# intellerce/controlanimate

Measured on AMD Instinct MI355X. Metric: frames_per_sec, higher is better.
Workload: dtype fp16

## Files before the change

### controlanimate_amd/attention.py

```python
from __future__ import annotations

from typing import Optional

import torch
from torch import nn

from . import kernels as K
from .attention_processor import Attention, AttnProcessor2_0
from .context import ExecCtx, dispatch
from .layers import HipConv1x1, HipGroupNorm, HipLayerNorm, HipLinear, LnFold, WeightArena, _f32, geglu_interleave, ln_fold_enabled


class GEGLU(nn.Module):
    def __init__(self, dim_in: int, dim_out: int):
        super().__init__()
        self.dim_in, self.dim_out = dim_in, dim_out
        self.proj = HipLinear(dim_in, dim_out * 2)
        self.w = self.b = None

    def pack(self, arena: WeightArena, dtype):
        self.w = arena.add((2 * self.dim_out, self.dim_in), dtype, lambda: geglu_interleave(_f32(self.proj.weight)))
        self.b = arena.add((2 * self.dim_out,), torch.float32, lambda: geglu_interleave(_f32(self.proj.bias)))

    def run(self, x: torch.Tensor) -> torch.Tensor:
        return K.gemm(x, self.w.t, bias=self.b.t, geglu=True)


class FeedForward(nn.Module):
    def __init__(self, dim: int, dim_out: Optional[int] = None, mult: int = 4, dropout: float = 0.0,
                 activation_fn: str = "geglu", final_dropout: bool = False):
        super().__init__()
        if activation_fn != "geglu":
            raise NotImplementedError(activation_fn)
        inner = int(dim * mult)
        self.net = nn.ModuleList([GEGLU(dim, inner), nn.Identity(), HipLinear(inner, dim_out or dim)])

    def pack(self, arena, dtype, fold_ln=None):
        self.fold = None
        if fold_ln is not None and ln_fold_enabled():
            self.fold = LnFold(arena, dtype, fold_ln, [self.net[0].proj], geglu=True)
        else:
            self.net[0].pack(arena, dtype)
        self.net[2].pack(arena, dtype)
        self.w2f = None
        out = self.net[2]
        if self.fold is not None and self.fold.w.frag is not None and (out.out_features, out.in_features) == (320, 1280):
            from .layers import frag_order2
            self.w2f = arena.add((320, 1280), dtype, lambda: frag_order2(out.weight.detach().float()))

    def run_with_proj_out(self, x: torch.Tensor, residual: Optional[torch.Tensor], proj_frag, proj_bias, proj_residual) -> Optional[torch.Tensor]:
        fold = getattr(self, "fold", None)
        if fold is None or getattr(self, "w2f", None) is None or proj_frag is None or not dispatch.attn_out_fused:
            return None
        return K.ff_fused(x, fold.w.frag[0].t, fold.b.t, fold.cs.t, self.w2f.t, None if self.net[2].b is None else self.net[2].b.t,
                          fold.eps, residual=residual, w_out_frag=proj_frag.t, bias_out=None if proj_bias is None else proj_bias.t,
                          residual_out=proj_residual)

    def run(self, x: torch.Tensor, residual: Optional[torch.Tensor] = None, sums=None) -> torch.Tensor:
        fold = getattr(self, "fold", None)
        if fold is not None and getattr(self, "w2f", None) is not None and sums is None:
            y = K.ff_fused(x, fold.w.frag[0].t, fold.b.t, fold.cs.t, self.w2f.t, None if self.net[2].b is None else self.net[2].b.t,
                           fold.eps, residual=residual)
            if y is not None:
                return y
        if fold is not None:
            h = K.gemm(x, fold.w.t, bias=fold.b.t, geglu=True, ln=(K.RowStats(x, fold.eps, sums), fold.cs.t))
        else:
            h = self.net[0].run(x)
        return self.net[2].run(h, residual=residual)


class BasicTransformerBlock(nn.Module):
    def __init__(self, query_dim: int, num_attention_heads: int, attention_head_dim: int, dropout=0.0,
                 cross_attention_dim: Optional[int] = None, activation_fn: str = "geglu", attention_bias: bool = False,
                 upcast_attention: bool = False, unet_use_cross_frame_attention=False, unet_use_temporal_attention=False, **_):
        super().__init__()
        if unet_use_cross_frame_attention or unet_use_temporal_attention:
            raise NotImplementedError("both flags are false in configs/inference/inference-v{1,2}.yaml")
        self.processor = AttnProcessor2_0()
        self.attn1 = Attention(query_dim, heads=num_attention_heads, dim_head=attention_head_dim, bias=attention_bias)
        self.norm1 = HipLayerNorm(query_dim)
        self.attn2 = Attention(query_dim, cross_attention_dim=cross_attention_dim, heads=num_attention_heads,
                               dim_head=attention_head_dim, bias=attention_bias) if cross_attention_dim is not None else None
        self.norm2 = HipLayerNorm(query_dim) if cross_attention_dim is not None else None
        self.ff = FeedForward(query_dim, activation_fn=activation_fn)
        self.norm3 = HipLayerNorm(query_dim)

    def get_processor(self, return_deprecated_lora: bool = False):
        return self.processor

    def set_processor(self, processor, _remove_lora: bool = False):
        if isinstance(getattr(self, "processor", None), nn.Module) and not isinstance(processor, nn.Module):
            self._modules.pop("processor", None)
        self.processor = processor

    def pack(self, arena, dtype):
        self.attn1.pack(arena, dtype, fold_ln=self.norm1)
        self.norm1.pack(arena, dtype)
        if self.attn2 is not None:
            self.attn2.pack(arena, dtype, fold_ln=self.norm2)
            self.norm2.pack(arena, dtype)
        self.ff.pack(arena, dtype, fold_ln=self.norm3)
        self.norm3.pack(arena, dtype)

    def forward(self, x: torch.Tensor, ctx: ExecCtx, proj_out=None) -> torch.Tensor:
        return self.forward_rest(self.forward_self(x), ctx, proj_out=proj_out)

    def forward_self(self, x: torch.Tensor) -> torch.Tensor:
        B, N, C = x.shape
        next_folded = (self.attn2.fold if self.attn2 is not None else self.ff.fold) is not None
        if self.attn1.fold is not None:
            x = self.attn1(x, residual=x, ln=(K.RowStats(x.view(B * N, C), self.norm1.eps, K.row_sums_of(x)), self.attn1.fold),
                           row_sums=next_folded)
        else:
            x = self.attn1(self.norm1.run(x.view(B * N, C)).view(B, N, C), residual=x, row_sums=next_folded)
        return x

    def forward_rest(self, x: torch.Tensor, ctx: ExecCtx, proj_out=None) -> torch.Tensor:
        B, N, C = x.shape
        if self.attn2 is not None:
            kw = dict(encoder_hidden_states=ctx.ehs, residual=x, frames_per_kv=ctx.frames_per_kv, kv_mod=ctx.kv_mod, cache=ctx.cache,
                      row_sums=self.ff.fold is not None)
            if self.attn2.fold is not None:
                x = self.attn2(x, ln=(K.RowStats(x.view(B * N, C), self.norm2.eps, K.row_sums_of(x)), self.attn2.fold), **kw)
            else:
                x = self.attn2(self.norm2.run(x.view(B * N, C)).view(B, N, C), **kw)
        x2 = x.view(B * N, C)
        if self.ff.fold is None:
            return self.ff.run(self.norm3.run(x2), residual=x2).view(B, N, C)
        if proj_out is not None and K.row_sums_of(x) is None:
            y = self.ff.run_with_proj_out(x2, x2, *proj_out)
            if y is not None:
                y = y.view(B, N, C)
                y._proj_out_done = True
                return y
        return self.ff.run(x2, residual=x2, sums=K.row_sums_of(x)).view(B, N, C)


class Transformer3DModel(nn.Module):
    def __init__(self, num_attention_heads: int = 16, attention_head_dim: int = 88, in_channels: Optional[int] = None,
                 num_layers: int = 1, norm_num_groups: int = 32, cross_attention_dim: Optional[int] = None,
                 use_linear_projection: bool = False, **kw):
        super().__init__()
        if use_linear_projection:
            raise NotImplementedError("SD1.5 uses 1x1-conv projections")
        inner = num_attention_heads * attention_head_dim
        self.in_channels = in_channels
        self.norm = HipGroupNorm(norm_num_groups, in_channels, eps=1e-6)
        self.proj_in = HipConv1x1(in_channels, inner)
        self.transformer_blocks = nn.ModuleList([
            BasicTransformerBlock(inner, num_attention_heads, attention_head_dim, cross_attention_dim=cross_attention_dim, **kw)
            for _ in range(num_layers)])
        self.proj_out = HipConv1x1(inner, in_channels)

    def pack(self, arena, dtype):
        self.norm.pack(arena, dtype)
        self.proj_in.pack(arena, dtype)
        for b in self.transformer_blocks:
            b.pack(arena, dtype)
        self.proj_out.pack(arena, dtype)
        self.proj_out_frag = None
        po = self.proj_out
        if tuple(po.weight.shape[:2]) == (320, 320) and getattr(self.transformer_blocks[-1].ff, "w2f", None) is not None:
            from .layers import frag_order_wout
            self.proj_out_frag = arena.add((102400,), dtype, lambda: frag_order_wout(_f32(po.weight).reshape(320, 320)))

    def forward(self, x: torch.Tensor, ctx: ExecCtx, shared_half: bool = False) -> torch.Tensor:
        images, h, w, c = x.shape
        rows = images * h * w
        y = self.norm.run(x)
        y0 = self.proj_in.run(y.view(rows, c), row_sums=self.transformer_blocks[0].attn1.fold is not None)
        y = K.carry_row_sums(y0.view(images, h * w, -1), y0)
        nblk = len(self.transformer_blocks)
        pfrag = getattr(self, "proj_out_frag", None)

        def proj(k, x_rows):
            return (pfrag, self.proj_out.b, x_rows) if (k == nblk - 1 and pfrag is not None) else None
        if shared_half:
            y = self.transformer_blocks[0].forward_self(y)
            y, x = K.repeat_batch(y), K.repeat_batch(x)
            images, rows = 2 * images, 2 * rows
            y = self.transformer_blocks[0].forward_rest(y, ctx, proj_out=proj(0, x.view(rows, c)))
        for k in range(1 if shared_half else 0, nblk):
            y = self.transformer_blocks[k](y, ctx, proj_out=proj(k, x.view(rows, c)))
        if getattr(y, "_proj_out_done", False):
            return y.view(images, h, w, c)
        return self.proj_out.run(y.view(rows, -1), residual=x.view(rows, c)).view(images, h, w, c)
```

### controlanimate_amd/context.py

```python
from __future__ import annotations

from dataclasses import dataclass, field
from typing import Optional

import torch


@dataclass
class ExecCtx:
    b: int
    f: int
    dtype: torch.dtype
    temb: torch.Tensor
    emb_groups: int
    ehs: Optional[torch.Tensor] = None
    frames_per_kv: int = 1
    kv_mod: int = 0
    gn_frames_per_stat: int = 1
    cache: dict = field(default_factory=dict)

    @property
    def images(self) -> int:
        return self.b * self.f

    def rows_per_emb_group(self, h: int, w: int) -> int:
        return self.images // self.emb_groups * h * w


class Dispatch:
    gemm_ar = True
    ff_fused = True
    tattn_fused = True
    xattn_fused = True
    attn_out_fused = True
    xattn_ip_fused = True
    conv_winograd = True
    gn_winograd = True
    conv_up2_phase = True
    ln_row_sums = True
    repeat_kernel = True
    ln_fold = True
    cfg_shared = True
    cn_cfg_dedup = True
    pdc_block_fused = True
    dpt_head_fused = False
    pose_conv7_direct = True
    nbae_refine_fused = True
    controlnet_streams = 2


dispatch = Dispatch()
```

### controlanimate_amd/csrc/ca_gemm_plan.h

```cpp
#pragma once
#include "ca_gemm_core.h"

namespace ca_gemm_detail {

inline unsigned desc_bytes(int64_t elems) {
  const int64_t b = elems * 2;
  return (b > 0 && b < (int64_t)0xFFFFFF00ll) ? (unsigned)b : 0u;
}

inline bool dma_shape_ok(const GemmKParams& p) { return (p.c1 + p.c2) % BK == 0 && (p.c2 == 0 || p.c1 % BK == 0); }
inline bool dma_sizes_ok(const GemmKParams& p) { return p.a_bytes != 0 && p.w_bytes != 0 && (p.c2 == 0 || p.a2_bytes != 0); }
inline bool dma_capable(const GemmKParams& p) { return dma_shape_ok(p) && dma_sizes_ok(p); }

inline bool wres_eligible(const GemmKParams& p) {
  static const int wres_env = CA_KNOB("CA_GEMM_WRES", -1);
  const int kc = p.c1 + p.c2;
  return wres_env != 0 && kc == 320 && p.taps == 1 && (p.c2 == 0 || p.c1 % 32 == 0) && p.n % 160 == 0 && p.n / 160 <= 32 && !p.out_f32 &&
         p.splits <= 1 && !p.ln_parts && dma_sizes_ok(p) &&
         (!p.rowbias || p.rows_per_group % 32 == 0) &&
         act_out_fit31(p) &&
         (wres_env == 1 || p.m >= 16384);
}

inline bool ar_eligible(const GemmKParams& p, bool scratch) {
  static const int ar_env = CA_KNOB("CA_GEMM_AR", -1);
  if (ar_env == 0 || !p.wf || !wres_eligible(p)) return false;
  return p.c2 == 0 && p.n % 64 == 0 && p.alpha == 1.f && p.post == 1.f && p.act == CA_ACT_NONE && !p.row_sums && ((uintptr_t)p.wf & 15) == 0 &&
         ((uintptr_t)p.c & 15) == 0 && p.ldc % 8 == 0 && (!p.res || (((uintptr_t)p.res & 15) == 0 && p.ld_res % 8 == 0 && !p.geglu && !p.ln_colsum)) &&
         (!p.rowbias || (p.rows_per_group % 128 == 0 && !p.geglu)) && (!p.ln_inline || scratch) &&
         (ar_env == 1 || p.n >= 960);
}

struct GemmPlan {
  PlanKind kind;
  int bm, bn, nbuf;
  int splits;
  unsigned tiles;
};

inline bool ps_capable(const GemmKParams& p) {
  const int nt = p.taps * p.kc_tiles;
  const bool fits32 = act_out_fit31(p) && p.w_bytes < FIT31;
  const bool aligned = ((uintptr_t)p.c & 15) == 0 && (!p.res || ((uintptr_t)p.res & 15) == 0) && p.ldc % 8 == 0 && (!p.res || p.ld_res % 8 == 0);
  return dma_capable(p) && p.n % 320 == 0 && nt >= 2 && p.splits <= 1 && !p.out_f32 && !p.ln_inline && (p.ln_parts <= 2 || p.ln_parts == 4) && fits32 && aligned &&
         (!p.rowbias || p.rows_per_group % 64 == 0) && !(p.geglu && (p.res || p.row_sums)) && p.post == 1.f && p.act == CA_ACT_NONE;
}

inline bool pq_capable(const GemmKParams& p, int mode) {
  const bool conv_ok = mode != 1 || (p.pad_lo == 1 && p.ups == 0 && p.hin >= 2 && p.win >= 2 && (int64_t)(p.m / (p.hout * p.wout) + 1) * p.hin * p.win < (1 << 23) &&
                                     (p.hout - 1) * p.stride < p.hin && (p.wout - 1) * p.stride < p.win);
  const bool epi1 = p.geglu || p.ln_colsum || p.ln_stats;
  return ps_capable(p) && (!p.row_sums || (mode == 0 && !epi1)) && (mode == 1 || p.c2 == 0) && (!p.rowbias || p.rows_per_group % 128 == 0) && conv_ok &&
         (!epi1 || (mode == 0 && !p.res && !p.rowbias && p.ln_parts == 0 && (!p.ln_colsum || p.ln_stats)));
}

struct SplitKRule { int env, max_blocks; bool f32_out; };
struct SplitK { int ranges; int64_t bytes; };
inline SplitK splitk_decide(const GemmKParams& p, int mode) {
  static const SplitKRule conv{CA_KNOB("CA_SPLITK", -1), 383, true}, dense{CA_KNOB("CA_SPLITK_DENSE", -1), 192, false};
  const SplitKRule& r = mode == 0 ? dense : conv;
  const SplitK none{1, 0};
  if (!dma_capable(p) || p.ln_inline || p.row_sums || p.ln_parts) return none;
  if (r.env == 0 || p.geglu || (p.out_f32 && !r.f32_out) || p.n % 128 != 0) return none;
  const int nt = p.taps * p.kc_tiles;
  const int64_t blocks = (int64_t)ceil_div_i(p.m, 128) * (p.n / 128);
  if (blocks > r.max_blocks || nt < 48) return none;
  int s = r.env > 0 ? r.env : (int)((960 + blocks - 1) / blocks);
  if (s > 8) s = 8;
  while (s > 1 && nt / s < 12) --s;
  return s > 1 ? SplitK{s, (int64_t)s * p.m * p.n * 4} : none;
}
inline void splitk_apply(const SplitK& k, void* workspace, int64_t workspace_bytes, GemmKParams& p) {
  if (k.ranges > 1 && workspace && workspace_bytes >= k.bytes) {
    p.splits = k.ranges;
    p.partial = reinterpret_cast<float*>(workspace);
  }
}

inline GemmPlan plan_gemm(const GemmKParams& p, int mode) {
  const bool dma = dma_capable(p);
  const int nt = p.taps * p.kc_tiles;
  if (dma && p.splits > 1) {
    static const int pp_split_env = CA_KNOB("CA_SPLITK_PP", 1);
    if (pp_split_env && mode == 0 && p.n % 320 == 0) {
      const int tiles320 = ceil_div_i(p.m, 128) * (p.n / 320);
      int s_eff = 256 / tiles320;
      if (s_eff > p.splits) s_eff = p.splits;
      if (s_eff >= 2 && tiles320 * s_eff >= 128 && nt / s_eff >= 12) {
        return GemmPlan{PK_PP2_SPLITK, 128, 320, 0, s_eff, (unsigned)tiles320};
      }
    }
    return GemmPlan{PK_DMA_SPLITK, 128, 128, 1, p.splits, (unsigned)(ceil_div_i(p.m, 128) * (p.n / 128))};
  }
  static const int pp_env = CA_KNOB("CA_GEMM_PP", -1);
  static const int pq_env = CA_KNOB("CA_GEMM_PQ", -1);
  if (pq_env != 0 && pq_capable(p, mode)) {
    const int64_t tiles = (int64_t)ceil_div_i(p.m, 256) * (p.n / 320);
    const bool dflt = mode == 1 ? (tiles >= 256 && (p.n >= 640 || nt >= 64)) : (tiles >= 256 && (tiles % 256 == 0 || tiles >= 1024) && nt >= 8 && !wres_eligible(p));
    const bool epi1 = p.geglu || p.ln_colsum || p.ln_stats;
    const bool dflt2 = dflt && (mode == 1 || p.geglu), dflt3 = dflt && mode == 1, dflt4 = dflt && (mode == 1 || p.geglu || !epi1);
    if ((pq_env < 0 && dflt) || pq_env == 1 || (pq_env == 2 && dflt2) || (pq_env == 3 && dflt3) || (pq_env == 4 && dflt4) || (pq_env == 5 && dflt)) {
      return GemmPlan{PK_PQ, 256, 320, 0, 1, (unsigned)tiles};
    }
  }
  static const int ps_env = CA_KNOB("CA_GEMM_PS", -1);
  if (ps_env != 0 && ps_capable(p)) {
    const int64_t tiles = (int64_t)ceil_div_i(p.m, 128) * (p.n / 320);
    const bool dflt = mode == 0 && !wres_eligible(p) && nt <= 20 && tiles >= 256 && (p.geglu || p.n <= 1280);
    if ((ps_env < 0 && dflt) || ps_env == 1 || (ps_env == 2 && !(mode == 0 && wres_eligible(p)))) {
      return GemmPlan{PK_PS, 128, 320, 0, 1, (unsigned)tiles};
    }
  }
  if (mode == 0 && dma && ar_eligible(p, p.partial != nullptr)) return GemmPlan{PK_AR, 128, 64, 0, 1, 0u};
  if (mode == 0 && dma && wres_eligible(p)) return GemmPlan{PK_WRES, 256, 160, 0, 1, 0u};
  if (dma && pp_env != 0 && nt >= 2 && p.n % 320 == 0 && p.splits <= 1) {
    const int64_t tiles = (int64_t)ceil_div_i(p.m, 128) * (p.n / 320);
    if (p.row_sums || pp_env == 2 || (pp_env < 0 && tiles >= 128 && nt >= 10 && (tiles <= 256 || (tiles <= 512 && mode == 0)))) {
      return GemmPlan{PK_PP2, 128, 320, 0, 1, (unsigned)tiles};
    }
  }
  const bool wide = p.n % 128 == 0 && (int64_t)ceil_div_i(p.m, 128) * ceil_div_i(p.n, 128) >= 512;
  const int64_t blocks = (int64_t)ceil_div_i(p.m, 128) * ceil_div_i(p.n, wide ? 128 : 64);
  const int nbuf = blocks >= 512 ? 1 : 3;
  if (dma && !wide && p.n % 160 == 0 && (int64_t)ceil_div_i(p.m, 128) * (p.n / 160) >= 512) return GemmPlan{PK_DMA, 128, 160, 1, 1, 0u};
  return GemmPlan{dma ? PK_DMA : PK_REG, 128, wide ? 128 : 64, dma ? nbuf : 2, 1, 0u};
}

inline int row_sums_parts_of(GemmKParams p) {
  p.row_sums = nullptr;
  if (p.geglu || p.out_f32) return 0;
  const PlanKind k = plan_gemm(p, 0).kind;
// ... 236 lines not shown
```

### controlanimate_amd/csrc/ca_gemm_pp.hip

```cpp
#include "ca_gemm_core.h"
#include <type_traits>

namespace {
using namespace ca_gemm_detail;
#include "ca_gemm_pp2.h"
#include "ca_gemm_wres.h"
#include "ca_gemm_ps.h"
#include "ca_gemm_pq.h"

int cu_count() {
  static int n = 0;
  if (!n) {
    int dev = 0;
    hipDeviceProp_t prop;
    if (hipGetDevice(&dev) == hipSuccess && hipGetDeviceProperties(&prop, dev) == hipSuccess) n = prop.multiProcessorCount;
    if (n <= 0) n = 256;
  }
  return n;
}

template <class Launch>
int launch_stamped(const GemmKParams& p, hipStream_t st, const char* label, unsigned sep, unsigned eol, Launch launch) {
  static unsigned long long* dbuf = nullptr;
  if (!dbuf && hipMalloc(&dbuf, 4096 * 8) != hipSuccess) return CA_ERR_LAUNCH;
  (void)hipMemsetAsync(dbuf, 0, 4096 * 8, st);
  GemmKParams q = p;
  q.partial = reinterpret_cast<float*>(dbuf);
  launch(q);
  (void)hipStreamSynchronize(st);
  static int printed = 0;
  if (printed++ < 1) {
    static unsigned long long host[4096];
    (void)hipMemcpy(host, dbuf, sizeof(host), hipMemcpyDeviceToHost);
    for (int g = 0; g < 2; ++g) {
      fprintf(stderr, "[%s stamps group %d, %dx%dx%d] tag:delta_cycles ...\n", label, g, p.m, p.n, (p.c1 + p.c2) * p.taps);
      unsigned long long prev = host[g * 2048];
      for (int i = 0; i < 1000 && host[g * 2048 + 2 * i]; ++i) {
        fprintf(stderr, "%llu:%llu ", host[g * 2048 + 2 * i + 1], host[g * 2048 + 2 * i] - prev);
        prev = host[g * 2048 + 2 * i];
        if (host[g * 2048 + 2 * i + 1] == sep) fprintf(stderr, "| ");
        if (host[g * 2048 + 2 * i + 1] == eol) fprintf(stderr, "\n");
      }
      fprintf(stderr, "\n");
    }
  }
  return CA_OK;
}

template <int DT, int MODE>
int launch_pp(const GemmKParams& p, PlanKind kind, unsigned tiles, hipStream_t st) {
  const unsigned c_bytes = (unsigned)c_extent_bytes(p), res_bytes = (unsigned)res_extent_bytes(p);
  const unsigned grid = tiles < (unsigned)cu_count() ? tiles : (unsigned)cu_count();
  switch (kind) {
    case PK_PQ: {
      auto launch = [&](const GemmKParams& q) {
        if (MODE == 0 && (q.geglu || q.ln_colsum || q.ln_stats)) hipLaunchKernelGGL((k_gemm_pq<DT, 0, 1>), dim3(grid), dim3(512), 0, st, q, (int)tiles, c_bytes, 0u);
        else if (MODE == 0 && q.row_sums) hipLaunchKernelGGL((k_gemm_pq<DT, 0, 2>), dim3(grid), dim3(512), 0, st, q, (int)tiles, c_bytes, res_bytes);
        else hipLaunchKernelGGL((k_gemm_pq<DT, MODE>), dim3(grid), dim3(512), 0, st, q, (int)tiles, c_bytes, res_bytes);
      };
#ifdef CA_STAMPS
      if (p.dbg == 9) return launch_stamped(p, st, "pq", 8, 10, launch);
#endif
      launch(p);
      return CA_OK;
    }
    case PK_PS: {
      auto launch = [&](const GemmKParams& q) { hipLaunchKernelGGL((k_gemm_ps<DT, MODE>), dim3(grid), dim3(512), 0, st, q, (int)tiles, c_bytes, res_bytes); };
#ifdef CA_STAMPS
      if (p.dbg == 9) return launch_stamped(p, st, "ps", 8, 10, launch);
#endif
      launch(p);
      return CA_OK;
    }
    case PK_WRES: {
      if (MODE != 0) return CA_ERR_LAUNCH;
      const int panels = p.n / 160;
      const int chunks = (p.m + 255) / 256;
      int per = (cu_count() / 8) / panels;
      if (per * 8 > chunks) per = chunks / 8;
      if (per < 1) per = 1;
      const unsigned rb_bytes = p.rowbias ? (unsigned)(((int64_t)((p.m - 1) / p.rows_per_group) * p.ld_rowbias + p.n) * 4) : 16u;
      hipLaunchKernelGGL((k_gemm_wres<DT>), dim3(8 * per * panels), dim3(512), 0, st, p, panels, 8 * per, chunks, rb_bytes, c_bytes, res_bytes);
      return CA_OK;
    }
    case PK_PP2:
      hipLaunchKernelGGL((k_gemm_pp2<DT, MODE>), dim3(tiles), dim3(512), 0, st, p);
      return CA_OK;
// ... 21 lines not shown
```

### controlanimate_amd/csrc/ca_gemm_pq.h

```cpp

#ifdef CA_PQ_ABLATE
#define CA_PQ_ABL(bit) (((CA_PQ_ABLATE) & (bit)) != 0)
#else
#define CA_PQ_ABL(bit) false
#endif

__device__ __forceinline__ unsigned pq_udiv(unsigned r, unsigned d, unsigned mag) {
  const unsigned q = __umulhi(r, mag);
  return r - q * d >= d ? q + 1 : q;
}

template <int DT, int MODE, int EPI = 0>
__global__ __launch_bounds__(512, 2) void k_gemm_pq(GemmKParams p, int tiles_total, unsigned c_bytes, unsigned res_bytes) {
  constexpr int BM = 256, BN = 320, KT = 64;
  constexpr int TM = 8, TN = 5;
  constexpr int A_ROWS = 256, B0_ROWS = 128, B1_ROWS = 192;
  constexpr int OFF_A = 0, OFF_B0 = A_ROWS * KT, OFF_B1 = (A_ROWS + B0_ROWS) * KT;
  constexpr int BUF = (A_ROWS + B0_ROWS + B1_ROWS) * KT;
  constexpr int PAR_BASE = 2 * BUF * 2;
  constexpr int P_BI = 0, P_RB0 = 1280, P_RB1 = 2560, P_CS = 3840, PSET = EPI == 1 ? 5120 : 4096;
  constexpr int FLAG_BASE = PAR_BASE + 2 * PSET;
  constexpr int SMEM_BYTES = FLAG_BASE + 8 * 2 * 256;
  static_assert(SMEM_BYTES <= 160 * 1024, "LDS");
  __shared__ __attribute__((aligned(16))) unsigned char smem_b[SMEM_BYTES];
// ... 23 lines not shown
  const bool geglu = EPI == 1 && p.geglu != 0;
  const unsigned long long res_addr = (unsigned long long)(p.res ? (const void*)p.res : (const void*)p.c);
  const u32x4 rs_res = {(unsigned)__builtin_amdgcn_readfirstlane((int)(unsigned)res_addr), (unsigned)__builtin_amdgcn_readfirstlane((int)(unsigned)((res_addr >> 32) & 0xffffu)),
                        (unsigned)__builtin_amdgcn_readfirstlane((int)(p.res ? res_bytes : 0u)), 0x00020000u};
  const unsigned rb_groups = p.rowbias ? (unsigned)((p.m + p.rows_per_group - 1) / p.rows_per_group) : 0u;
  const __amdgpu_buffer_rsrc_t rs_rb = __builtin_amdgcn_make_buffer_rsrc((void*)(p.rowbias ? (const void*)p.rowbias : (const void*)p.w), 0,
                                                                         p.rowbias ? (unsigned)(((int64_t)(rb_groups - 1) * p.ld_rowbias + p.n) * 4) : 0u, 0x00020000);
  const __amdgpu_buffer_rsrc_t rs_seq = __builtin_amdgcn_make_buffer_rsrc((void*)ca_seq_table.v, 0, 4096u, 0x00020000);

#ifdef CA_STAMPS
  unsigned long long* const stamps = reinterpret_cast<unsigned long long*>(p.partial);
  int stamp_i = 0;
  auto stamp = [&](int tag) __attribute__((always_inline)) {
    if (p.dbg == 9 && blockIdx.x == 0 && (wid == 0 || wid == 4) && lane == 0 && stamp_i < 1000) {
      stamps[(wid >> 2) * 2048 + 2 * stamp_i] = __builtin_readcyclecounter();
      stamps[(wid >> 2) * 2048 + 2 * stamp_i + 1] = (unsigned long long)tag;
      ++stamp_i;
    }
  };
#else
  auto stamp = [&](int) __attribute__((always_inline)) {};
#endif
  auto swz = [](int row) { return (row >> 1) & 7; };
  const int kc = p.c1 + p.c2;
  const int kct = kc / KT;
  const unsigned wld = (unsigned)(p.taps * kc);
  const int nt = p.taps * kct;
  const int total_kt = my_tiles * nt;

  constexpr unsigned OOB_V = 0x80000000u;
  unsigned b0_v[2] = {0, 0}, b1_v[3] = {0, 0, 0};
  unsigned a_v[4] = {0, 0, 0, 0};
  int d_seq = 0, d_t = 0, d_tap = 0, d_c0 = 0, d_n = 0;
  bool d_live = true;
  unsigned char* const my_flags = smem_b + FLAG_BASE + wid * 2 * 256;

  auto tile_of = [&](int seq, int& tm, int& tn) __attribute__((always_inline)) -> bool {
    const int id = seq * G + bslot;
    if (id >= tiles_total) return false;
    tile_coords((unsigned)id, tiles_m, tiles_n, tm, tn);
    return true;
  };

  auto dma_set_tile = [&](int seq, int m0, int n0) __attribute__((always_inline)) {
    if (CA_PQ_ABL(16)) m0 = 0, n0 = 0;
    int lane_o = lane;
    asm volatile("" : "+v"(lane_o));
    const int r8 = lane_o >> 3, cp = lane_o & 7;
    const int a_chunk0 = cp ^ swz(r8), b1_chunk0 = cp ^ swz(wid * 24 + r8);
#pragma unroll
    for (int i = 0; i < 4; ++i) {
      const int m = m0 + wid * 32 + i * 8 + r8;
      const bool ok = m < p.m;
      if (MODE == 2) {
        const int ph = m0 / (p.up2_tiles * BM);
        const int py = ph >> 1, px = ph & 1;
        const int r = m - ph * (p.up2_tiles * BM);
        const bool okr = r < p.up2_rows;
        const int rr = okr ? r : p.up2_rows - 1;
        const unsigned q = pq_udiv((unsigned)rr, (unsigned)p.win, p.up2_mag_w);
        const int xs = rr - (int)q * p.win;
        const int ys = (int)q - (int)pq_udiv(q, (unsigned)p.hin, p.up2_mag_h) * p.hin;
        const int hi0 = ys + py - 1, wi0 = xs + px - 1;
        const int p0 = rr + (py - 1) * p.win + (px - 1);
        a_v[i] = ((unsigned)p0 & 0xFFFFFFu) | (hi0 >= 0 ? 1u << 24 : 0u) | (hi0 + 1 < p.hin ? 1u << 25 : 0u) | (wi0 >= 0 ? 1u << 26 : 0u) | (wi0 + 1 < p.win ? 1u << 27 : 0u) |
                 (okr ? 1u << 28 : 0u);
      } else if (MODE == 1) {
        const int mm = ok ? m : p.m - 1;
        const int hw = p.hout * p.wout;
        const int img = mm / hw;
        const int rem = mm - img * hw;
        const int ho = rem / p.wout, wo = rem - ho * p.wout;
        const int hi0 = ho * p.stride - p.pad_lo, wi0 = wo * p.stride - p.pad_lo;
        const int p0 = (img * p.hin + hi0) * p.win + wi0;
        a_v[i] = ((unsigned)p0 & 0xFFFFFFu) | (hi0 >= 0 ? 1u << 24 : 0u) | (hi0 + 2 < p.hin ? 1u << 25 : 0u) | (wi0 >= 0 ? 1u << 26 : 0u) | (wi0 + 2 < p.win ? 1u << 27 : 0u) |
                 (ok ? 1u << 28 : 0u);
      } else {
        a_v[i] = ok ? (unsigned)m * (unsigned)p.lda * 2u + (unsigned)((a_chunk0 ^ (4 * (i & 1))) * 16) : OOB_V;
      }
    }
    unsigned wgrp = 0u;
    if (MODE == 0 && EPI == 0 && p.w_group_rows > 0) wgrp = (unsigned)(m0 / p.w_group_rows) * p.w_group_stride;
    if (MODE == 2) wgrp = (unsigned)(m0 / (p.up2_tiles * BM)) * p.w_group_stride;
#pragma unroll
    for (int i = 0; i < 2; ++i) {
      const int r = wid * 16 + i * 8 + r8;
      b0_v[i] = wgrp + (unsigned)(n0 + (r >> 5) * 80 + ca_ps_col((r >> 4) & 1, r & 15, geglu)) * wld * 2u + (unsigned)((a_chunk0 ^ (4 * i)) * 16);
    }
#pragma unroll
    for (int i = 0; i < 3; ++i) {
      const int r1 = wid * 24 + i * 8 + r8;
      b1_v[i] = wgrp + (unsigned)(n0 + (r1 / 48) * 80 + ca_ps_col(2 + (r1 % 48) / 16, r1 & 15, geglu)) * wld * 2u + (unsigned)((b1_chunk0 ^ (4 * (i & 1))) * 16);
    }
    d_tap = 0;
    d_c0 = 0;
    unsigned char* pset = smem_b + PAR_BASE + (seq & 1) * PSET;
    if (EPI == 1 && wid == 4) {
      const __amdgpu_buffer_rsrc_t rs_cs = __builtin_amdgcn_make_buffer_rsrc((void*)(p.ln_colsum ? (const void*)p.ln_colsum : (const void*)p.w), 0, p.ln_colsum ? (unsigned)p.n * 4u : 0u, 0x00020000);
      __builtin_amdgcn_raw_ptr_buffer_load_lds(rs_cs, (__attribute__((address_space(3))) void*)(pset + P_CS), 16, (unsigned)n0 * 4u + lane_o * 16u, 0, 0, 0);
      __builtin_amdgcn_raw_ptr_buffer_load_lds(rs_cs, (__attribute__((address_space(3))) void*)(pset + P_CS + 1024), 4, (unsigned)n0 * 4u + 1024u + lane_o * 4u, 0, 0, 0);
    }
    if (wid >= 1 && wid <= 3) {
      const bool has1 = p.rowbias && m0 / p.rows_per_group + 1 < (int)rb_groups;
      const unsigned base = wid == 1 ? (unsigned)n0 * 4u
                                     : wid == 2 ? (unsigned)n0 * 4u + (unsigned)(p.rowbias ? m0 / p.rows_per_group : 0) * (unsigned)p.ld_rowbias * 4u
                                                : (has1 ? (unsigned)n0 * 4u + (unsigned)(m0 / p.rows_per_group + 1) * (unsigned)p.ld_rowbias * 4u : OOB_V);
      unsigned char* dst = pset + (wid == 1 ? P_BI : wid == 2 ? P_RB0 : P_RB1);
      if (wid == 1) {
        __builtin_amdgcn_raw_ptr_buffer_load_lds(rs_bi, (__attribute__((address_space(3))) void*)dst, 16, base + lane_o * 16u, 0, 0, 0);
        __builtin_amdgcn_raw_ptr_buffer_load_lds(rs_bi, (__attribute__((address_space(3))) void*)(dst + 1024), 4, base + 1024u + lane_o * 4u, 0, 0, 0);
      } else {
        __builtin_amdgcn_raw_ptr_buffer_load_lds(rs_rb, (__attribute__((address_space(3))) void*)dst, 16, base + lane_o * 16u, 0, 0, 0);
        __builtin_amdgcn_raw_ptr_buffer_load_lds(rs_rb, (__attribute__((address_space(3))) void*)(dst + 1024), 4, base + 1024u + lane_o * 4u, 0, 0, 0);
      }
    }
  };

  auto issue_tile = [&]() __attribute__((always_inline)) {
    if (!d_live) return;
    if (CA_PQ_ABL(1) && d_n >= 2) {
      ++d_n;
      ++d_t;
      return;
    }
    const int par = d_n & 1;
    u16* buf = smem + par * BUF;
    const unsigned wk = (unsigned)(d_tap * kc + d_c0) * 2u;
    const bool src2 = d_c0 >= p.c1;
    __builtin_amdgcn_raw_ptr_buffer_load_lds(rs_w, (__attribute__((address_space(3))) void*)(buf + OFF_B0 + (wid * 2 + 0) * 8 * KT), 16, b0_v[0], wk, 0, 0);
    __builtin_amdgcn_raw_ptr_buffer_load_lds(rs_w, (__attribute__((address_space(3))) void*)(buf + OFF_B0 + (wid * 2 + 1) * 8 * KT), 16, b0_v[1], wk, 0, 0);
    if (MODE != 0) {
      int lane_o = lane;
      asm volatile("" : "+v"(lane_o));
      const unsigned cs2 = (unsigned)(src2 ? p.c2 : p.c1) * 2u;
      const int kh = MODE == 2 ? d_tap >> 1 : (d_tap >= 6 ? 2 : (d_tap >= 3 ? 1 : 0)), kw = MODE == 2 ? d_tap & 1 : d_tap - kh * 3;
      const unsigned need = MODE == 2 ? (1u << 28) | (kh == 0 ? 1u << 24 : 1u << 25) | (kw == 0 ? 1u << 26 : 1u << 27)
                                      : (1u << 28) | (kh == 0 ? 1u << 24 : kh == 2 ? 1u << 25 : 0u) | (kw == 0 ? 1u << 26 : kw == 2 ? 1u << 27 : 0u);
      const int delta = kh * p.win + kw;
      const unsigned cadd = (unsigned)(src2 ? d_c0 - p.c1 : d_c0) * 2u + (unsigned)(((lane_o & 7) ^ swz(lane_o >> 3)) * 16);
#pragma unroll
      for (int i = 0; i < 4; ++i) {
        const unsigned av = a_v[i];
        const int pix = (((int)(av << 8)) >> 8) + delta;
        const unsigned off = __umul24((unsigned)pix, cs2) + (cadd ^ ((i & 1) ? 64u : 0u));
        const unsigned voff = (av & need) == need ? off : OOB_V;
        void* d = buf + OFF_A + (wid * 4 + i) * 8 * KT;
        if (src2) __builtin_amdgcn_raw_ptr_buffer_load_lds(rs_a2, (__attribute__((address_space(3))) void*)d, 16, voff, 0, 0, 0);
        else __builtin_amdgcn_raw_ptr_buffer_load_lds(rs_a, (__attribute__((address_space(3))) void*)d, 16, voff, 0, 0, 0);
      }
    } else {
#pragma unroll
      for (int i = 0; i < 4; ++i)
        __builtin_amdgcn_raw_ptr_buffer_load_lds(rs_a, (__attribute__((address_space(3))) void*)(buf + OFF_A + (wid * 4 + i) * 8 * KT), 16, a_v[i], (unsigned)d_c0 * 2u, 0, 0);
    }
#pragma unroll
    for (int i = 0; i < 3; ++i)
      __builtin_amdgcn_raw_ptr_buffer_load_lds(rs_w, (__attribute__((address_space(3))) void*)(buf + OFF_B1 + (wid * 3 + i) * 8 * KT), 16, b1_v[i], wk, 0, 0);
    __builtin_amdgcn_raw_ptr_buffer_load_lds(rs_seq, (__attribute__((address_space(3))) void*)(my_flags + par * 256), 4, 0u, (unsigned)(d_n & 1023) * 4u, 0, 0);
    ++d_n;
    ++d_t;
    if (p.taps == 1) {
      d_c0 += KT;
    } else if (++d_tap == p.taps) {
      d_tap = 0;
      d_c0 += KT;
    }
  };
#define CA_PQ_SET_TILE(SEQ)                                  \
  {                                                          \
    int tm_, tn_;                                            \
    d_live = tile_of((SEQ), tm_, tn_);                       \
    if (d_live) dma_set_tile((SEQ), tm_ * BM, tn_ * BN);     \
  }
  auto advance_and_issue = [&]() __attribute__((always_inline)) {
    if (d_t == nt) {
      d_t = 0;
      ++d_seq;
      CA_PQ_SET_TILE(d_seq)
    }
    issue_tile();
  };
// ... 305 lines not shown
```

### controlanimate_amd/layers.py

```python
from __future__ import annotations

from typing import Callable, List, Optional, Sequence, Tuple

import torch
from torch import nn

from . import kernels as K
from .context import dispatch

ALIGN = 256


class Packed:

    __slots__ = ("shape", "dtype", "fill", "offset", "t", "frag")

    def __init__(self, shape, dtype, fill):
        self.shape = tuple(int(s) for s in shape)
        self.dtype = dtype
        self.fill = fill
        self.offset = -1
        self.t: Optional[torch.Tensor] = None
        self.frag = None

# ... 242 lines not shown
        def w_cat():
            return torch.cat([_f32(m.weight).reshape(m.weight.shape[0], -1) for m in mods], 0)

        def w_fold():
            w = w_cat() * _f32(ln.weight)[None, :]
            return geglu_interleave(w) if geglu else w

        def bias():
            b = w_cat() @ _f32(ln.bias)
            b = b + torch.cat([_f32(m.bias) if getattr(m, "bias", None) is not None else torch.zeros(m.weight.shape[0], device=m.weight.device) for m in mods], 0)
            return geglu_interleave(b) if geglu else b

        self.w = arena.add((n, k), dtype, w_fold)
        self.w_fold = w_fold
        if frag_wanted(n, k):
            self.w.frag = (arena.add((n, k), dtype, lambda: frag_order(w_fold(), geglu)), geglu)
        self.cs = arena.add((n,), torch.float32, lambda: w_fold().to(dtype).float().sum(1))
        self.b = arena.add((n,), torch.float32, bias)
        self.pe = None
        if pe is not None:
            self.pe = arena.add((pe.shape[-2], n), torch.float32, lambda: _f32(pe).reshape(pe.shape[-2], k).to(mods[0].weight.device) @ w_cat().to(dtype).float().t())
        self._rb_cache = {}

    def rowbias(self, b: int, f: int) -> torch.Tensor:
        if f > self.pe.t.shape[0]:
            raise ValueError(f"video_length {f} exceeds temporal_position_encoding_max_len {self.pe.t.shape[0]}")
        key = (b, f, self.pe.t.data_ptr())
        rb = self._rb_cache.get(key)
        if rb is None:
            rb = self._rb_cache[key] = self.pe.t[:f].repeat(b, 1).contiguous()
        return rb


def geglu_interleave(w: torch.Tensor) -> torch.Tensor:
    d = w.shape[0] // 2
    return torch.stack([w[:d], w[d:]], dim=1).reshape(w.shape)
```

### controlanimate_amd/motion_module.py

```python
from __future__ import annotations

import math

import torch
from torch import nn

from . import kernels as K
from .attention import FeedForward
from .attention_processor import Attention
from .context import ExecCtx
from .layers import HipGroupNorm, HipLayerNorm, HipLinear, WeightArena, _f32


def get_motion_module(in_channels, motion_module_type: str, motion_module_kwargs: dict):
    if motion_module_type == "Vanilla":
        return VanillaTemporalModule(in_channels=in_channels, **motion_module_kwargs)
    raise ValueError(motion_module_type)


class PositionalEncoding(nn.Module):
    def __init__(self, d_model, dropout=0.0, max_len=24):
        super().__init__()
        position = torch.arange(max_len).unsqueeze(1)
        div_term = torch.exp(torch.arange(0, d_model, 2) * (-math.log(10000.0) / d_model))
# ... 29 lines not shown
        no_bias = all(getattr(m, "bias", None) is None for m in (self.to_q, self.to_k, self.to_v))
        if self.fold is not None and pe is not None and no_bias and (self.heads, self.inner_dim, self.query_dim) == (8, 320, 320):
            from .layers import _f32, frag_order_tattn
            self.tfrag = arena.add((368640,), dtype, lambda: frag_order_tattn(torch.cat([_f32(m.weight) for m in (self.to_q, self.to_k, self.to_v)], 0)))
            self.tgamma = arena.add((320,), torch.float32, lambda: _f32(fold_ln.weight))
            self.tbias_pe = arena.add((pe.shape[-2], 320), torch.float32,
                                      lambda: _f32(pe).reshape(pe.shape[-2], 320).to(fold_ln.bias.device) + _f32(fold_ln.bias)[None, :])
            self.tln_eps = fold_ln.eps

    def pos_table(self, frames: int):
        if self.pos_encoder is None:
            return None
        if frames > self.pos_encoder.max_len:
            raise ValueError(f"video_length {frames} exceeds temporal_position_encoding_max_len {self.pos_encoder.max_len}")
        return self.pos_encoder.table.t[:frames]


class TemporalTransformerBlock(nn.Module):
    def __init__(self, dim, num_attention_heads, attention_head_dim, attention_block_types=("Temporal_Self", "Temporal_Self"),
                 dropout=0.0, cross_attention_dim=768, activation_fn="geglu", attention_bias=False, upcast_attention=False,
                 cross_frame_attention_mode=None, temporal_position_encoding=False, temporal_position_encoding_max_len=24, **_):
        super().__init__()
        self.attention_blocks = nn.ModuleList([
            VersatileAttention(attention_mode=name.split("_")[0],
                               cross_attention_dim=cross_attention_dim if name.endswith("_Cross") else None,
                               query_dim=dim, heads=num_attention_heads, dim_head=attention_head_dim, bias=attention_bias,
                               temporal_position_encoding=temporal_position_encoding,
                               temporal_position_encoding_max_len=temporal_position_encoding_max_len)
            for name in attention_block_types])
        self.norms = nn.ModuleList([HipLayerNorm(dim) for _ in attention_block_types])
        self.ff = FeedForward(dim, activation_fn=activation_fn)
        self.ff_norm = HipLayerNorm(dim)

    def pack(self, arena, dtype):
        for attn, norm in zip(self.attention_blocks, self.norms):
            attn.pack(arena, dtype, fold_ln=norm)
            norm.pack(arena, dtype)
        self.ff.pack(arena, dtype, fold_ln=self.ff_norm)
        self.ff_norm.pack(arena, dtype)

    def forward(self, x: torch.Tensor, ctx: ExecCtx, tokens: int, proj_out=None) -> torch.Tensor:
        rows, C = x.shape
        nblk = len(self.attention_blocks)
        for i, (attn, norm) in enumerate(zip(self.attention_blocks, self.norms)):
            nxt = (self.attention_blocks[i + 1].fold if i + 1 < nblk else self.ff.fold) is not None
            if attn.fold is not None:
                o = attn(x.view(1, rows, C), residual=x.view(1, rows, C), temporal=(ctx.b, ctx.f, tokens),
                         ln=(K.RowStats(x, norm.eps, K.row_sums_of(x)), attn.fold), row_sums=nxt)
            else:
                n = norm.run(x, pos=attn.pos_table(ctx.f), rows_per_frame=tokens, frames=ctx.f)
                o = attn(n.view(1, rows, C), residual=x.view(1, rows, C), temporal=(ctx.b, ctx.f, tokens), row_sums=nxt)
            x = K.carry_row_sums(o.view(rows, C), o)
        if self.ff.fold is None:
            return self.ff.run(self.ff_norm.run(x), residual=x)
        if proj_out is not None and K.row_sums_of(x) is None:
            y = self.ff.run_with_proj_out(x, x, *proj_out)
            if y is not None:
                y._proj_out_done = True
                return y
        return self.ff.run(x, residual=x, sums=K.row_sums_of(x))


class TemporalTransformer3DModel(nn.Module):
    def __init__(self, in_channels, num_attention_heads, attention_head_dim, num_layers, norm_num_groups=32, **kw):
        super().__init__()
        inner = num_attention_heads * attention_head_dim
        self.norm = HipGroupNorm(norm_num_groups, in_channels, eps=1e-6)
        self.proj_in = HipLinear(in_channels, inner)
        self.transformer_blocks = nn.ModuleList([
            TemporalTransformerBlock(dim=inner, num_attention_heads=num_attention_heads,
                                     attention_head_dim=attention_head_dim, **kw) for _ in range(num_layers)])
        self.proj_out = HipLinear(inner, in_channels)

    def pack(self, arena, dtype):
        self.norm.pack(arena, dtype)
        self.proj_in.pack(arena, dtype)
        for b in self.transformer_blocks:
            b.pack(arena, dtype)
        self.proj_out.pack(arena, dtype)
        self.proj_out_frag = None
        po = self.proj_out
        if tuple(po.weight.shape) == (320, 320) and getattr(self.transformer_blocks[-1].ff, "w2f", None) is not None:
            from .layers import frag_order_wout
            self.proj_out_frag = arena.add((102400,), dtype, lambda: frag_order_wout(_f32(po.weight)))

    def forward(self, x: torch.Tensor, ctx: ExecCtx) -> torch.Tensor:
        images, h, w, c = x.shape
        rows = images * h * w
        y = self.norm.run(x)
        y = self.proj_in.run(y.view(rows, c), row_sums=self.transformer_blocks[0].attention_blocks[0].fold is not None)
        pfrag = getattr(self, "proj_out_frag", None)
        last = len(self.transformer_blocks) - 1
        for k, blk in enumerate(self.transformer_blocks):
            y = blk(y, ctx, h * w, proj_out=(pfrag, self.proj_out.b, x.view(rows, c)) if (k == last and pfrag is not None) else None)
        if getattr(y, "_proj_out_done", False):
            return y.view(images, h, w, c)
        return self.proj_out.run(y, residual=x.view(rows, c)).view(images, h, w, c)


class VanillaTemporalModule(nn.Module):
    def __init__(self, in_channels, num_attention_heads=8, num_transformer_block=2,
                 attention_block_types=("Temporal_Self", "Temporal_Self"), cross_frame_attention_mode=None,
                 temporal_position_encoding=False, temporal_position_encoding_max_len=24, temporal_attention_dim_div=1,
                 zero_initialize=True):
        super().__init__()
        self.temporal_transformer = TemporalTransformer3DModel(
            in_channels=in_channels, num_attention_heads=num_attention_heads,
            attention_head_dim=in_channels // num_attention_heads // temporal_attention_dim_div,
            num_layers=num_transformer_block, attention_block_types=attention_block_types,
            cross_frame_attention_mode=cross_frame_attention_mode, temporal_position_encoding=temporal_position_encoding,
            temporal_position_encoding_max_len=temporal_position_encoding_max_len)
        if zero_initialize:
            nn.init.zeros_(self.temporal_transformer.proj_out.weight)
            nn.init.zeros_(self.temporal_transformer.proj_out.bias)

    def pack(self, arena, dtype):
        self.temporal_transformer.pack(arena, dtype)

    def forward(self, x: torch.Tensor, ctx: ExecCtx) -> torch.Tensor:
        return self.temporal_transformer(x, ctx)
```

Measured before the change: 16.12.

## Fold feed-forward output linear into transformer proj_out as one two-source GEMM

For the last transformer block, whenever the fused 320-channel path does not apply, the FF output projection and the following proj_out linear are merged algebraically into a single GEMM. It uses weights [Wp·W2 | Wp] over the concatenated inputs (GEGLU output, FF residual) and the folded bias Wp·b2+bp. This drops one full GEMM launch and the round trip of its intermediate activation. To support it, the persistent PQ GEMM kernel gains a second-A-source load path for non-epilogue mode 0, with launch guards and a heuristic gate for two-source cases. The catch is a larger K dimension (inner+C instead of inner) for that GEMM, plus fp16 rounding differences from the premultiplied weights.

```diff
diff --git a/controlanimate_amd/attention.py b/controlanimate_amd/attention.py
--- a/controlanimate_amd/attention.py
+++ b/controlanimate_amd/attention.py
@@ -8,7 +8,7 @@
 from . import kernels as K
 from .attention_processor import Attention, AttnProcessor2_0
 from .context import ExecCtx, dispatch
-from .layers import HipConv1x1, HipGroupNorm, HipLayerNorm, HipLinear, LnFold, WeightArena, _f32, geglu_interleave, ln_fold_enabled
+from .layers import FfProjFold, HipConv1x1, HipGroupNorm, HipLayerNorm, HipLinear, LnFold, WeightArena, _f32, geglu_interleave, ln_fold_enabled
 
 
 class GEGLU(nn.Module):
@@ -35,22 +35,31 @@
         inner = int(dim * mult)
         self.net = nn.ModuleList([GEGLU(dim, inner), nn.Identity(), HipLinear(inner, dim_out or dim)])
 
-    def pack(self, arena, dtype, fold_ln=None):
-        self.fold = None
+    def pack(self, arena, dtype, fold_ln=None, proj_out=None):
+        self.fold = self.pfold = None
         if fold_ln is not None and ln_fold_enabled():
             self.fold = LnFold(arena, dtype, fold_ln, [self.net[0].proj], geglu=True)
         else:
             self.net[0].pack(arena, dtype)
+        out = self.net[2]
+        c320 = self.fold is not None and self.fold.w.frag is not None and (out.out_features, out.in_features) == (320, 1280)
+        if proj_out is not None and self.fold is not None and not c320 and dispatch.ff_proj_fold:
+            self.pfold = FfProjFold(arena, dtype, out, proj_out)
+            out.w = out.b = None
+            self.w2f = None
+            return
         self.net[2].pack(arena, dtype)
         self.w2f = None
-        out = self.net[2]
-        if self.fold is not None and self.fold.w.frag is not None and (out.out_features, out.in_features) == (320, 1280):
+        if c320:
             from .layers import frag_order2
             self.w2f = arena.add((320, 1280), dtype, lambda: frag_order2(out.weight.detach().float()))
 
-    def run_with_proj_out(self, x: torch.Tensor, residual: Optional[torch.Tensor], proj_frag, proj_bias, proj_residual) -> Optional[torch.Tensor]:
+    def run_with_proj_out(self, x: torch.Tensor, residual: Optional[torch.Tensor], proj_frag, proj_bias, proj_residual, sums=None) -> Optional[torch.Tensor]:
         fold = getattr(self, "fold", None)
-        if fold is None or getattr(self, "w2f", None) is None or proj_frag is None or not dispatch.attn_out_fused:
+        if getattr(self, "pfold", None) is not None:
+            g = K.gemm(x, fold.w.t, bias=fold.b.t, geglu=True, ln=(K.RowStats(x, fold.eps, sums), fold.cs.t))
+            return self.pfold.run(g, residual, proj_residual)
+        if fold is None or getattr(self, "w2f", None) is None or proj_frag is None or not dispatch.attn_out_fused or sums is not None:
             return None
         return K.ff_fused(x, fold.w.frag[0].t, fold.b.t, fold.cs.t, self.w2f.t, None if self.net[2].b is None else self.net[2].b.t,
                           fold.eps, residual=residual, w_out_frag=proj_frag.t, bias_out=None if proj_bias is None else proj_bias.t,
@@ -58,6 +67,8 @@
 
     def run(self, x: torch.Tensor, residual: Optional[torch.Tensor] = None, sums=None) -> torch.Tensor:
         fold = getattr(self, "fold", None)
+        if getattr(self, "pfold", None) is not None:
+            raise RuntimeError("this feed-forward's output projection was packed together with proj_out: run_with_proj_out")
         if fold is not None and getattr(self, "w2f", None) is not None and sums is None:
             y = K.ff_fused(x, fold.w.frag[0].t, fold.b.t, fold.cs.t, self.w2f.t, None if self.net[2].b is None else self.net[2].b.t,
                            fold.eps, residual=residual)
@@ -94,13 +105,13 @@
             self._modules.pop("processor", None)
         self.processor = processor
 
-    def pack(self, arena, dtype):
+    def pack(self, arena, dtype, proj_out=None):
         self.attn1.pack(arena, dtype, fold_ln=self.norm1)
         self.norm1.pack(arena, dtype)
         if self.attn2 is not None:
             self.attn2.pack(arena, dtype, fold_ln=self.norm2)
             self.norm2.pack(arena, dtype)
-        self.ff.pack(arena, dtype, fold_ln=self.norm3)
+        self.ff.pack(arena, dtype, fold_ln=self.norm3, proj_out=proj_out)
         self.norm3.pack(arena, dtype)
 
     def forward(self, x: torch.Tensor, ctx: ExecCtx, proj_out=None) -> torch.Tensor:
@@ -128,10 +139,10 @@
         x2 = x.view(B * N, C)
         if self.ff.fold is None:
             return self.ff.run(self.norm3.run(x2), residual=x2).view(B, N, C)
-        if proj_out is not None and K.row_sums_of(x) is None:
-            y = self.ff.run_with_proj_out(x2, x2, *proj_out)
+        if proj_out is not None:
+            y = self.ff.run_with_proj_out(x2, x2, *proj_out, sums=K.row_sums_of(x))
             if y is not None:
-                y = y.view(B, N, C)
+                y = y.view(B, N, -1)
                 y._proj_out_done = True
                 return y
         return self.ff.run(x2, residual=x2, sums=K.row_sums_of(x)).view(B, N, C)
@@ -156,9 +167,13 @@
     def pack(self, arena, dtype):
         self.norm.pack(arena, dtype)
         self.proj_in.pack(arena, dtype)
-        for b in self.transformer_blocks:
-            b.pack(arena, dtype)
-        self.proj_out.pack(arena, dtype)
+        nblk = len(self.transformer_blocks)
+        for k, b in enumerate(self.transformer_blocks):
+            b.pack(arena, dtype, proj_out=self.proj_out if k == nblk - 1 else None)
+        if self.transformer_blocks[-1].ff.pfold is not None:
+            self.proj_out.w = self.proj_out.b = None
+        else:
+            self.proj_out.pack(arena, dtype)
         self.proj_out_frag = None
         po = self.proj_out
         if tuple(po.weight.shape[:2]) == (320, 320) and getattr(self.transformer_blocks[-1].ff, "w2f", None) is not None:
@@ -173,9 +188,10 @@
         y = K.carry_row_sums(y0.view(images, h * w, -1), y0)
         nblk = len(self.transformer_blocks)
         pfrag = getattr(self, "proj_out_frag", None)
+        absorbed = getattr(self.transformer_blocks[-1].ff, "pfold", None) is not None
 
         def proj(k, x_rows):
-            return (pfrag, self.proj_out.b, x_rows) if (k == nblk - 1 and pfrag is not None) else None
+            return (pfrag, self.proj_out.b, x_rows) if (k == nblk - 1 and (pfrag is not None or absorbed)) else None
         if shared_half:
             y = self.transformer_blocks[0].forward_self(y)
             y, x = K.repeat_batch(y), K.repeat_batch(x)
diff --git a/controlanimate_amd/context.py b/controlanimate_amd/context.py
--- a/controlanimate_amd/context.py
+++ b/controlanimate_amd/context.py
@@ -40,6 +40,7 @@
     ln_row_sums = True
     repeat_kernel = True
     ln_fold = True
+    ff_proj_fold = True
     cfg_shared = True
     cn_cfg_dedup = True
     pdc_block_fused = True
diff --git a/controlanimate_amd/csrc/ca_gemm_plan.h b/controlanimate_amd/csrc/ca_gemm_plan.h
--- a/controlanimate_amd/csrc/ca_gemm_plan.h
+++ b/controlanimate_amd/csrc/ca_gemm_plan.h
@@ -50,7 +50,7 @@
   const bool conv_ok = mode != 1 || (p.pad_lo == 1 && p.ups == 0 && p.hin >= 2 && p.win >= 2 && (int64_t)(p.m / (p.hout * p.wout) + 1) * p.hin * p.win < (1 << 23) &&
                                      (p.hout - 1) * p.stride < p.hin && (p.wout - 1) * p.stride < p.win);
   const bool epi1 = p.geglu || p.ln_colsum || p.ln_stats;
-  return ps_capable(p) && (!p.row_sums || (mode == 0 && !epi1)) && (mode == 1 || p.c2 == 0) && (!p.rowbias || p.rows_per_group % 128 == 0) && conv_ok &&
+  return ps_capable(p) && (!p.row_sums || (mode == 0 && !epi1)) && (mode == 1 || p.c2 == 0 || !epi1) && (!p.rowbias || p.rows_per_group % 128 == 0) && conv_ok &&
          (!epi1 || (mode == 0 && !p.res && !p.rowbias && p.ln_parts == 0 && (!p.ln_colsum || p.ln_stats)));
 }
 
@@ -96,7 +96,8 @@
   static const int pq_env = CA_KNOB("CA_GEMM_PQ", -1);
   if (pq_env != 0 && pq_capable(p, mode)) {
     const int64_t tiles = (int64_t)ceil_div_i(p.m, 256) * (p.n / 320);
-    const bool dflt = mode == 1 ? (tiles >= 256 && (p.n >= 640 || nt >= 64)) : (tiles >= 256 && (tiles % 256 == 0 || tiles >= 1024) && nt >= 8 && !wres_eligible(p));
+    const bool two_src_ok = p.c2 == 0 || mode == 1 || (nt > 20 && p.n == 640);
+    const bool dflt = mode == 1 ? (tiles >= 256 && (p.n >= 640 || nt >= 64)) : (tiles >= 256 && (tiles % 256 == 0 || tiles >= 1024) && nt >= 8 && !wres_eligible(p) && two_src_ok);
     const bool epi1 = p.geglu || p.ln_colsum || p.ln_stats;
     const bool dflt2 = dflt && (mode == 1 || p.geglu), dflt3 = dflt && mode == 1, dflt4 = dflt && (mode == 1 || p.geglu || !epi1);
     if ((pq_env < 0 && dflt) || pq_env == 1 || (pq_env == 2 && dflt2) || (pq_env == 3 && dflt3) || (pq_env == 4 && dflt4) || (pq_env == 5 && dflt)) {
diff --git a/controlanimate_amd/csrc/ca_gemm_pp.hip b/controlanimate_amd/csrc/ca_gemm_pp.hip
--- a/controlanimate_amd/csrc/ca_gemm_pp.hip
+++ b/controlanimate_amd/csrc/ca_gemm_pp.hip
@@ -53,6 +53,7 @@
   const unsigned grid = tiles < (unsigned)cu_count() ? tiles : (unsigned)cu_count();
   switch (kind) {
     case PK_PQ: {
+      if (p.c2 != 0 && (p.c1 % 64 != 0 || p.c2 % 64 != 0 || !p.a2 || (MODE == 0 && (p.geglu || p.ln_colsum || p.ln_stats)))) return CA_ERR_LAUNCH;
       auto launch = [&](const GemmKParams& q) {
         if (MODE == 0 && (q.geglu || q.ln_colsum || q.ln_stats)) hipLaunchKernelGGL((k_gemm_pq<DT, 0, 1>), dim3(grid), dim3(512), 0, st, q, (int)tiles, c_bytes, 0u);
         else if (MODE == 0 && q.row_sums) hipLaunchKernelGGL((k_gemm_pq<DT, 0, 2>), dim3(grid), dim3(512), 0, st, q, (int)tiles, c_bytes, res_bytes);
diff --git a/controlanimate_amd/csrc/ca_gemm_pq.h b/controlanimate_amd/csrc/ca_gemm_pq.h
--- a/controlanimate_amd/csrc/ca_gemm_pq.h
+++ b/controlanimate_amd/csrc/ca_gemm_pq.h
@@ -79,6 +79,7 @@
   unsigned b0_v[2] = {0, 0}, b1_v[3] = {0, 0, 0};
   unsigned a_v[4] = {0, 0, 0, 0};
   int d_seq = 0, d_t = 0, d_tap = 0, d_c0 = 0, d_n = 0;
+  int d_m0 = 0;
   bool d_live = true;
   unsigned char* const my_flags = smem_b + FLAG_BASE + wid * 2 * 256;
 
@@ -141,6 +142,7 @@
     }
     d_tap = 0;
     d_c0 = 0;
+    if (MODE == 0 && EPI != 1) d_m0 = m0 + wid * 32;
     unsigned char* pset = smem_b + PAR_BASE + (seq & 1) * PSET;
     if (EPI == 1 && wid == 4) {
       const __amdgpu_buffer_rsrc_t rs_cs = __builtin_amdgcn_make_buffer_rsrc((void*)(p.ln_colsum ? (const void*)p.ln_colsum : (const void*)p.w), 0, p.ln_colsum ? (unsigned)p.n * 4u : 0u, 0x00020000);
@@ -194,6 +196,18 @@
         void* d = buf + OFF_A + (wid * 4 + i) * 8 * KT;
         if (src2) __builtin_amdgcn_raw_ptr_buffer_load_lds(rs_a2, (__attribute__((address_space(3))) void*)d, 16, voff, 0, 0, 0);
         else __builtin_amdgcn_raw_ptr_buffer_load_lds(rs_a, (__attribute__((address_space(3))) void*)d, 16, voff, 0, 0, 0);
+      }
+    } else if (EPI != 1 && src2) {
+      int lane_o = lane;
+      asm volatile("" : "+v"(lane_o));
+      const int r8 = lane_o >> 3;
+      const unsigned ch = (unsigned)(((lane_o & 7) ^ swz(r8)) * 16);
+      const unsigned ak = (unsigned)(d_c0 - p.c1) * 2u;
+#pragma unroll
+      for (int i = 0; i < 4; ++i) {
+        const int m = d_m0 + i * 8 + r8;
+        const unsigned voff = m < p.m ? (unsigned)m * (unsigned)p.lda2 * 2u + (ch ^ ((i & 1) ? 64u : 0u)) : OOB_V;
+        __builtin_amdgcn_raw_ptr_buffer_load_lds(rs_a2, (__attribute__((address_space(3))) void*)(buf + OFF_A + (wid * 4 + i) * 8 * KT), 16, voff, ak, 0, 0);
       }
     } else {
 #pragma unroll
diff --git a/controlanimate_amd/layers.py b/controlanimate_amd/layers.py
--- a/controlanimate_amd/layers.py
+++ b/controlanimate_amd/layers.py
@@ -298,6 +298,41 @@
         return rb
 
 
+def ff_proj_fold_operands(w2, b2, wp, bp, acc=torch.float32):
+    wp = wp.detach().to(acc).reshape(wp.shape[0], -1)
+    w2 = w2.detach().to(acc)
+    b = wp.new_zeros(wp.shape[0]) if bp is None else bp.detach().to(acc).clone()
+    if b2 is not None:
+        b = b + wp @ b2.detach().to(acc)
+    return torch.cat([wp @ w2, wp], 1), b
+
+
+class FfProjFold:
+
+    def __init__(self, arena: WeightArena, dtype, ff_out: "HipLinear", proj_out: nn.Module):
+        self.ff_out, self.proj_out = ff_out, proj_out
+        n, inner = proj_out.weight.shape[0], ff_out.in_features
+        assert ff_out.out_features == proj_out.weight.shape[1]
+        self._ops = None
+
+        def w_fill():
+            self._ops = self.operands()
+            return self._ops[0]
+
+        def b_fill():
+            ops, self._ops = self._ops, None
+            return ops[1]
+
+        self.w = arena.add((n, inner + ff_out.out_features), dtype, w_fill)
+        self.b = arena.add((n,), torch.float32, b_fill)
+
+    def operands(self, acc=torch.float32):
+        return ff_proj_fold_operands(self.ff_out.weight, self.ff_out.bias, self.proj_out.weight, self.proj_out.bias, acc)
+
+    def run(self, g: torch.Tensor, h2: torch.Tensor, x_in: torch.Tensor) -> torch.Tensor:
+        return K.gemm(g, self.w.t, a2=h2, bias=self.b.t, residual=x_in)
+
+
 def geglu_interleave(w: torch.Tensor) -> torch.Tensor:
     d = w.shape[0] // 2
     return torch.stack([w[:d], w[d:]], dim=1).reshape(w.shape)
diff --git a/controlanimate_amd/motion_module.py b/controlanimate_amd/motion_module.py
--- a/controlanimate_amd/motion_module.py
+++ b/controlanimate_amd/motion_module.py
@@ -85,11 +85,11 @@
         self.ff = FeedForward(dim, activation_fn=activation_fn)
         self.ff_norm = HipLayerNorm(dim)
 
-    def pack(self, arena, dtype):
+    def pack(self, arena, dtype, proj_out=None):
         for attn, norm in zip(self.attention_blocks, self.norms):
             attn.pack(arena, dtype, fold_ln=norm)
             norm.pack(arena, dtype)
-        self.ff.pack(arena, dtype, fold_ln=self.ff_norm)
+        self.ff.pack(arena, dtype, fold_ln=self.ff_norm, proj_out=proj_out)
         self.ff_norm.pack(arena, dtype)
 
     def forward(self, x: torch.Tensor, ctx: ExecCtx, tokens: int, proj_out=None) -> torch.Tensor:
@@ -106,8 +106,8 @@
             x = K.carry_row_sums(o.view(rows, C), o)
         if self.ff.fold is None:
             return self.ff.run(self.ff_norm.run(x), residual=x)
-        if proj_out is not None and K.row_sums_of(x) is None:
-            y = self.ff.run_with_proj_out(x, x, *proj_out)
+        if proj_out is not None:
+            y = self.ff.run_with_proj_out(x, x, *proj_out, sums=K.row_sums_of(x))
             if y is not None:
                 y._proj_out_done = True
                 return y
@@ -128,9 +128,13 @@
     def pack(self, arena, dtype):
         self.norm.pack(arena, dtype)
         self.proj_in.pack(arena, dtype)
-        for b in self.transformer_blocks:
-            b.pack(arena, dtype)
-        self.proj_out.pack(arena, dtype)
+        last = len(self.transformer_blocks) - 1
+        for k, b in enumerate(self.transformer_blocks):
+            b.pack(arena, dtype, proj_out=self.proj_out if k == last else None)
+        if self.transformer_blocks[-1].ff.pfold is not None:
+            self.proj_out.w = self.proj_out.b = None
+        else:
+            self.proj_out.pack(arena, dtype)
         self.proj_out_frag = None
         po = self.proj_out
         if tuple(po.weight.shape) == (320, 320) and getattr(self.transformer_blocks[-1].ff, "w2f", None) is not None:
@@ -144,8 +148,9 @@
         y = self.proj_in.run(y.view(rows, c), row_sums=self.transformer_blocks[0].attention_blocks[0].fold is not None)
         pfrag = getattr(self, "proj_out_frag", None)
         last = len(self.transformer_blocks) - 1
+        absorbed = getattr(self.transformer_blocks[-1].ff, "pfold", None) is not None
         for k, blk in enumerate(self.transformer_blocks):
-            y = blk(y, ctx, h * w, proj_out=(pfrag, self.proj_out.b, x.view(rows, c)) if (k == last and pfrag is not None) else None)
+            y = blk(y, ctx, h * w, proj_out=(pfrag, self.proj_out.b, x.view(rows, c)) if (k == last and (pfrag is not None or absorbed)) else None)
         if getattr(y, "_proj_out_done", False):
             return y.view(images, h, w, c)
         return self.proj_out.run(y, residual=x.view(rows, c)).view(images, h, w, c)
```

Result: no change. 16.27 (median of 6 runs) (+1.0%).
